# johannesulf/TabCorr

Hardware: AMD Instinct MI355X
Metric: predict_calls_per_sec (higher is better)
Workload: dtype f64; 1 GPU; BASELINE configs[1]: Zheng07 predict(), synthetic auto table 50 mass bins x {cen,sat} (G=100, P=5050), 19 rp bins, n_gauss_prim=10, batch of 10000 draws per GPU per step, draws and results resident in HBM; n_tables=1, gather=none, gather_payload=ngal + xi (160 B per draw), gather_every_steps=32, lanes=4, rccl_ranks=0

## Files before the change

tabcorr_amd/csrc/internal.h:

```cpp
#pragma once

#include <hip/hip_runtime.h>
#include <hip/hip_ext.h>

#include <algorithm>
#include <chrono>
#include <cmath>
#include <cstdarg>
#include <cstdio>
#include <cstdlib>
#include <cstring>
#include <map>
#include <memory>
#include <string>
#include <utility>
#include <vector>

#include "../../include/tabcorr_amd.h"
#include "../../include/tabcorr_amd_testing.h"
#include "fastmath.h"
#include "hostmath.h"
#include "kernel_args.h"

namespace tc {
// ... 188 lines not shown
    tried = false;
  }
};

inline int env_int(const char* name, int fallback) {
#ifdef TC_DEVELOPER_KNOBS
  const char* value = getenv(name);
  if (value == nullptr || *value == 0) return fallback;
  return atoi(value);
#else
  (void)name;
  return fallback;
#endif
}

struct Tuning {
  int lanes = 4;
  int pipeline = 1;
  int single_draw = 1;
  int many_blocks = 256;
  int single_round = 1;
  int poll_done = 1;
  int quad_waves = 0;
  int quad_waves_f32 = 3;
  int quad_merge = 1;
  int quad_order = -1;
  int prio_occ = 2, prio_contract = 1, prio_finalize = 3;
  int finalize_threads = 0;
  int finalize_row_blocks = 0;
  int occ_splits = 0;
  int occ_per_cu = 4;
  int n_groups = 0, n_waves = 0, lds_min = 0, min_chunk_entries = 32;
  int k_splits = 0;
  int trace = 0;
  int autotune_after = 0;
  int sync_chunks = 0;
  int sync_form = 32;
  int sync_stagger = 10;
  int sync_direct_out = 2;
  int async_direct_in = 1;
  int async_direct_out = 2;
  int series = -1;
  int cross_defer = 1;
  int fused_defer = 2;
  int fused_sat_cap = 6;
  int cross_wide_min_draws = 4096;
  int cross_target = 160;
  int resident_aperture = 1;
  int cross_min_draws = 192;
  int fused = 1;
  int fused_min_draws = 0;
  int fused_max_draws = 30720;
  int fused_waves = 0;
  int fused_draws = 0;
  int fused_spread = 1, fused_spread_min = 8192, fused_spread_rounds = 1;
  int prio_fused = 1, prio_fused_occ = 2, prio_fused_out = 3;
  int deterministic = 0;
  int skip_occ = 0, skip_finalize = 0;
  void load() {
    fused = env_int("TC_FUSED", fused);
    fused_min_draws = env_int("TC_FUSED_MIN_DRAWS", fused_min_draws);
    fused_max_draws = env_int("TC_FUSED_MAX_DRAWS", fused_max_draws);
    prio_fused = env_int("TC_PRIO_FUSED", prio_fused);
    prio_fused_occ = env_int("TC_PRIO_FUSED_OCC", prio_fused_occ);
    prio_fused_out = env_int("TC_PRIO_FUSED_OUT", prio_fused_out);
    lanes = env_int("TC_LANES", lanes);
    pipeline = env_int("TC_PIPELINE", pipeline);
    single_draw = env_int("TC_SINGLE_DRAW", single_draw);
    quad_waves = env_int("TC_QUAD_WAVES", quad_waves);
    quad_waves_f32 = env_int("TC_QUAD_WAVES_F32", quad_waves_f32);
    quad_merge = env_int("TC_QUAD_MERGE", quad_merge);
    prio_occ = env_int("TC_PRIO_O", prio_occ);
    prio_contract = env_int("TC_PRIO_C", prio_contract);
    prio_finalize = env_int("TC_PRIO_F", prio_finalize);
    finalize_threads = env_int("TC_FINALIZE_THREADS", finalize_threads);
    finalize_row_blocks = env_int("TC_FINALIZE_ROW_BLOCKS", finalize_row_blocks);
    occ_splits = env_int("TC_OCC_SPLITS", occ_splits);
    occ_per_cu = env_int("TC_OCC_PER_CU", occ_per_cu);
    n_groups = env_int("TC_NGROUPS", n_groups);
    n_waves = env_int("TC_NWAVES", n_waves);
    lds_min = env_int("TC_LDS_MIN", lds_min);
    min_chunk_entries = env_int("TC_MIN_CHUNK_ENTRIES", min_chunk_entries);
    k_splits = env_int("TC_KSPLITS", k_splits);
    trace = env_int("TC_TRACE", trace);
    skip_occ = env_int("TC_SKIP_OCC", skip_occ);
    skip_finalize = env_int("TC_SKIP_FINALIZE", skip_finalize);
  }
};

}
}

struct AutoChoice {
  static constexpr int kSizes = 9;
  static constexpr int64_t size(int i) { return (int64_t)256 << i; }
  int form[kSizes] = {};
  float us[kSizes][3] = {};
  int form_for(int64_t n_draws) const {
    if (n_draws <= size(0)) return form[0];
    if (n_draws >= size(kSizes - 1)) return form[kSizes - 1];
    int i = 0;
    while (size(i + 1) < n_draws) ++i;
    const double w = (double)(n_draws - size(i)) / (double)(size(i + 1) - size(i));
    static const int shape[3] = {0, 64, 32};
    int best = 0;
    double best_us = (1.0 - w) * us[i][0] + w * us[i + 1][0];
// ... 271 lines not shown
```

tabcorr_amd/csrc/kernels.hip.h:

```cpp
#pragma once

#include <hip/hip_runtime.h>

#include <cstdint>
#include <utility>

#include "fastmath.h"
#include "hostmath.h"
#include "kernel_args.h"
#include "series.h"

#ifdef TC_DEVELOPER_KNOBS
#define TC_TRACE(pointer) ((pointer) != nullptr)
#else
#define TC_TRACE(pointer) false
#endif

namespace tc {

static_assert(sizeof(QuadRun) == 32 && sizeof(QuadCompArgs) == 32, "read as 8 x int32");

typedef const __attribute__((address_space(4))) double* sc_f64;
typedef const __attribute__((address_space(4))) float* sc_f32;
typedef const __attribute__((address_space(4))) int32_t* sc_i32;
// ... 1857 lines not shown
    } else {
#pragma unroll
      for (int u = 0; u < UU; ++u) {
        const double av = u ? t.y : t.x;
        D[u][0] = __builtin_amdgcn_mfma_f64_16x16x4f64(av, b.x, D[u][0], 0, 0, 0);
        D[u][1] = __builtin_amdgcn_mfma_f64_16x16x4f64(av, b.y, D[u][1], 0, 0, 0);
      }
    }
  };
  fetch(t0, b0, cb);
  while (left > 0) {
    const int row_length = triangular ? rb + 1 : n_cb;
    const int n = row_length - cb < left ? row_length - cb : left;
    left -= n;
    f64x2 e[4];
#pragma unroll
    for (int v = 0; v < 4; ++v) e[v] = *(const f64x2*)(dens_e + (4 * rb + v) * DL);
    fetch(t1, b1, n > 1 ? cb + 1 : 0);
    __builtin_amdgcn_sched_barrier(0);
    mma(t0, b0, true);
    __builtin_amdgcn_sched_barrier(0);
    int t = 1;
    for (; t + 1 < n; t += 2) {
      fetch(t0, b0, cb + t + 1);
      __builtin_amdgcn_sched_barrier(0);
      mma(t1, b1, false);
      __builtin_amdgcn_sched_barrier(0);
      fetch(t1, b1, t + 2 < n ? cb + t + 2 : 0);
      __builtin_amdgcn_sched_barrier(0);
      mma(t0, b0, false);
      __builtin_amdgcn_sched_barrier(0);
    }
    if (t < n) {
      fetch(t0, b0, 0);
      __builtin_amdgcn_sched_barrier(0);
      mma(t1, b1, false);
      __builtin_amdgcn_sched_barrier(0);
    } else {
      t0 = t1;
      b0 = b1;
    }
#pragma unroll
    for (int u = 0; u < UU; ++u)
#pragma unroll
      for (int v = 0; v < 4; ++v) {
        F[u][0] = fma(D[u][0][v], e[v].x, F[u][0]);
        F[u][1] = fma(D[u][1][v], e[v].y, F[u][1]);
      }
    ++rb;
    cb = 0;
  }
}

__device__ __forceinline__ int wave_prefix_sum(int value) {
  auto shifted = [](int x, auto control, auto rows) {
    return __builtin_amdgcn_update_dpp(0, x, decltype(control)::value, decltype(rows)::value, 0xf,
                                       false);
  };
  typedef std::integral_constant<int, 0xf> all_rows;
  value += shifted(value, std::integral_constant<int, 0x111>(), all_rows());
  value += shifted(value, std::integral_constant<int, 0x112>(), all_rows());
  value += shifted(value, std::integral_constant<int, 0x114>(), all_rows());
  value += shifted(value, std::integral_constant<int, 0x118>(), all_rows());
  value += shifted(value, std::integral_constant<int, 0x142>(), std::integral_constant<int, 0xa>());
  value += shifted(value, std::integral_constant<int, 0x143>(), std::integral_constant<int, 0xc>());
  return value;
}

__device__ __forceinline__ double fused_quad_rows40(double select, double value, double sums) {
  return __builtin_amdgcn_mfma_f64_4x4x4f64(select, value, sums, 0, 0, 0);
}

template <int S0, int NS>
__device__ __forceinline__ void fused_quad_pass40(__amdgpu_buffer_rsrc_t rs_t, unsigned off_a,
                                                  unsigned unit_bytes, const double* dens_b,
                                                  const double* dens_e, int rb, int cb, int left,
                                                  bool triangular, int n_cb, unsigned unit_base,
                                                  double (&F)[NS][10]) {
  unsigned ua = (unit_base + (unsigned)(triangular ? rb * (rb + 1) / 2 + cb : rb * n_cb + cb)) *
                unit_bytes;
  double ta[2][NS];
  f64x2 tb[2][5];
  double D[NS][10];
  auto fetch = [&](int set, int column) {
#pragma unroll
    for (int s = 0; s < NS; ++s) {
      constexpr int kPairBytes = 1024;
      const int sub = S0 + s;
      const bool first_of_pair = (sub & 1) == 0 && s + 1 < NS;
      const bool second_of_pair = (sub & 1) == 1 && s >= 1;
      if (first_of_pair) {
        const f64x2 word = __builtin_bit_cast(
            f64x2, __builtin_amdgcn_raw_buffer_load_b128(rs_t, off_a + (sub / 2) * kPairBytes, ua,
                                                         0));
        ta[set][s] = word.x;
        ta[set][s + 1 < NS ? s + 1 : s] = word.y;
      } else if (!second_of_pair) {
        ta[set][s] = __builtin_bit_cast(
            double, __builtin_amdgcn_raw_buffer_load_b64(
                        rs_t, off_a + (sub / 2) * kPairBytes + (sub & 1) * 8, ua, 0));
      }
    }
#pragma unroll
    for (int q = 0; q < 5; ++q) tb[set][q] = *(const f64x2*)(dens_b + 4 * column * 40 + 2 * q);
    ua += unit_bytes;
  };
// ... 25 lines not shown
    const int n = row_length - cb < left ? row_length - cb : left;
    left -= n;
    f64x2 e[5];
#pragma unroll
    for (int q = 0; q < 5; ++q) e[q] = *(const f64x2*)(dens_e + 4 * rb * 40 + 2 * q);
    int t = 0;
    if (n > 1) {
      fetch(1, cb + 1);
      mma(0, true);
      fetch(0, 2 < n ? cb + 2 : 0);
      mma(1, false);
      t = 2;
    }
    for (; t + 1 < n; t += 2) {
      fetch(1, cb + t + 1);
      mma(0, false);
      fetch(0, t + 2 < n ? cb + t + 2 : 0);
      mma(1, false);
    }
    if (t < n) {
      fetch(1, 0);
      if (t == 0) mma(0, true); else mma(0, false);
#pragma unroll
      for (int s = 0; s < NS; ++s) ta[0][s] = ta[1][s];
#pragma unroll
      for (int q = 0; q < 5; ++q) tb[0][q] = tb[1][q];
    }
#pragma unroll
    for (int q = 0; q < 5; ++q)
#pragma unroll
      for (int s = 0; s < NS; ++s) {
        F[s][2 * q] = fma(D[s][2 * q], e[q].x, F[s][2 * q]);
        F[s][2 * q + 1] = fma(D[s][2 * q + 1], e[q].y, F[s][2 * q + 1]);
      }
    ++rb;
    cb = 0;
  }
}

template <int NGAUSS, int U, bool ASSEMBIAS, bool MODULATE, bool LEAUTHAUD = false,
          int W = kFusedWaves, int DL = 64, bool GROUPED = false, int SATDEFER = 0>
__global__ __launch_bounds__(64 * W, DL == 40 ? 2 : W == 8 ? (SATDEFER == 2 ? 4 : 2) : 1) void predict_fused_kernel(
    FusedArgs a) {
  static_assert(!SATDEFER || (NGAUSS == 10 && !ASSEMBIAS && !MODULATE && !LEAUTHAUD && DL != 32 &&
                              !GROUPED), "deferred pairs");
  static_assert(!GROUPED || (NGAUSS == 10 && !LEAUTHAUD), "groups of bins: Zheng07, ten nodes");
  static_assert((DL == 64 && (W == 8 || W == 16)) || ((DL == 32 || DL == 40) && W == 8),
                "workgroup shape");
  static_assert(DL == 64 || NGAUSS == 10 || LEAUTHAUD, "32 / 40 draws: ten nodes per bin");
  static_assert(DL != 40 || (!ASSEMBIAS && !MODULATE && !LEAUTHAUD && !GROUPED), "latency form");
  constexpr int PARTS = DL == 40 ? W : W * 32 / DL;
  static_assert(!LEAUTHAUD || (NGAUSS == 0 && !ASSEMBIAS), "Leauthaud11: any n_gauss, undecorated");
  constexpr int UP = (U + 1) / 2;
  extern __shared__ __attribute__((aligned(16))) double fused_lds[];
  constexpr int kSlotDoubles = fused_slot_doubles(W, DL);
  const int region_b = a.dens_rows * DL > kSlotDoubles ? a.dens_rows * DL : kSlotDoubles;
  double* dens = fused_lds;
  double* table = fused_lds + region_b;
  double(*red)[W][kLanes] = (double(*)[W][kLanes])(table + fm::kTableDoubles);
  const fm::Consts kc = fm::make_consts();
#ifdef TC_DEVELOPER_KNOBS
  const int skip = (a.priority >> 8) & 3;
  const int n_bins_occ = (skip & 1) ? 0 : a.n_bins;
  unsigned long long* const stamps =
      ((a.priority >> 10) & 1) && a.chi2 == nullptr ? (unsigned long long*)a.chi2_data : nullptr;
  auto wave_stamp = [&](int which) {
    if (stamps != nullptr && (threadIdx.x & 63) == 0 && W == 8 && ((threadIdx.x >> 6) & 3) == 0)
      stamps[blockIdx.x * 32 + 16 + 8 * (threadIdx.x >> 8) + which] =
          __builtin_amdgcn_s_memrealtime();
  };
  auto stamp = [&](int which) {
    if (stamps != nullptr && threadIdx.x == 0)
      stamps[blockIdx.x * 32 + which] = __builtin_amdgcn_s_memrealtime();
  };
  if (skip & 1)
    for (int idx = threadIdx.x; idx < a.n_bins * DL; idx += blockDim.x) fused_lds[idx] = 1e-3;
#else
  constexpr int skip = 0;
  const int n_bins_occ = a.n_bins;
  auto stamp = [](int) {};
  auto wave_stamp = [](int) {};
#endif
  stamp(0);
  set_priority((a.priority >> 2) & 3);
  const int lane = threadIdx.x & 63;
  const int wave = __builtin_amdgcn_readfirstlane(threadIdx.x >> 6);
  const int n_gauss = NGAUSS > 0 ? NGAUSS : a.n_gauss;
  {
    typedef double __attribute__((ext_vector_type(2))) double2v;
    const int hi = fm::kTableDoubles / 2;
    const double2v* src = (const double2v*)a.math_table;
    double2v* dst = (double2v*)table;
    for (int i = threadIdx.x; i < hi; i += blockDim.x) dst[i] = src[i];
  }
  for (int idx = a.n_bins * DL + threadIdx.x; idx < a.dens_rows * DL; idx += blockDim.x)
    dens[idx] = 0.0;
  __syncthreads();
  stamp(1);

  const int draw = DL != 32 ? lane : (lane & 31);
  const int half = DL != 32 ? 0 : (lane >> 5);
  const bool live = DL != 40 || lane < 40;
  auto dens_at = [&](int row, int d) -> double& {
    return dens[DL == 40 ? dens40(row, d) : row * DL + d];
  };
  const int64_t col = (int64_t)blockIdx.x * DL;
  const int64_t b0 = col + draw;
  const int64_t b = b0 < a.n_draws ? b0 : a.n_draws - 1;
  double norm;
  {
    const double* th = a.theta + b * a.n_theta;
    LeauthaudDraw ld;
    if (LEAUTHAUD) ld = prepare_leauthaud(table, kc, th);
    DrawParams dp = LEAUTHAUD ? prepare_draw(table, kc, 12.0, 1.0, 12.0, 13.0, 1.0, 0.0, 0.0)
                              : draw_params<ASSEMBIAS>(table, kc, th);
    series_setup<MODULATE>(dp, (GROUPED ? a.group.series : a.series) != nullptr && DL != 32,
                           (GROUPED ? a.group.sat_series : a.sat_series) != nullptr && DL != 32);
    sc_f64 log_m = (sc_f64)a.log_m;
    sc_f64 mass = (sc_f64)a.m;
    sc_f64 weight = (sc_f64)a.weight;
    sc_f64 weight_sum = weight + a.n_bins * n_gauss;
    sc_f64 n_h = (sc_f64)a.n_h;
    sc_f64 percentile = (sc_f64)a.percentile;
    const double f1 = (1.0 - a.split) / a.split, f2 = a.split / (1.0 - a.split);
    double sum_cen = 0.0, sum_sat = 0.0;
    stamp(2);
    if (GROUPED) {
      sc_i32 group_begin = (sc_i32)a.group.begin;
      sc_f64 n_h_m = (sc_f64)a.group.n_h;
      const GroupConsts gq{(sc_f64)a.group.log_m, (sc_f64)a.group.m, (sc_f64)a.group.weight,
                           (sc_f64)a.group.weight + a.n_bins * 10, (sc_f64)a.group.percentile,
                           (sc_i32)a.group.member,
                           SeriesConsts{(sc_f64)a.group.series, (sc_i32)a.group.series_thr,
                                        (sc_f64)a.group.sat_series,
                                        (sc_i32)a.group.sat_series_thr}};
      for (int gr = wave; gr < a.n_groups; gr += W) {
        const bool central = gr < a.n_central_groups;
        auto emit = [&](int mi, int g, double acc) {
          const double value = acc * n_h_m[mi];
          if (half == 0) dens[g * DL + draw] = value;
          if (central) sum_cen += value; else sum_sat += value;
        };
        if (DL == 32)
          occ_group_zheng07_halves<ASSEMBIAS, MODULATE>(
              table, kc, gr, group_begin[gr], group_begin[gr + 1], central, half, a.group.log_m,
              a.group.m, a.group.weight, gq, a.split, dp, emit);
        else
          occ_group_zheng07<ASSEMBIAS, MODULATE>(table, kc, gr, group_begin[gr],
                                                 group_begin[gr + 1], central, gq, a.split, dp,
                                                 emit);
      }
    }
    unsigned mine = 0;
    for (int g = wave; g < (GROUPED ? 0 : n_bins_occ); g += W) {
      const bool central = g < a.n_central;
      const bool above = ASSEMBIAS ? percentile[g] > a.split : false;
      bool deferred = false;
      const double acc =
          SATDEFER == 2 && central
              ? occ_cen_record(table, kc,
                               (sc_f64)a.cen_records + g * series::cen_record::kStride, dp,
                               &deferred) :
          SATDEFER && !central && (SATDEFER == 2 || a.sat_cap == series::sat::kShortest)
              ? occ_sat_record(table, kc,
                               (sc_f64)a.sat_records + g * series::sat_record::kStride, dp,
                               &deferred) :
          DL == 32 && LEAUTHAUD
              ? occ_bin_leauthaud11_halves<MODULATE>(table, kc, g, central, half, a.log_m, a.m,
                                                     a.weight, ld)
          : DL == 32  ? occ_bin_zheng07_halves<ASSEMBIAS, MODULATE>(table, kc, g, central, above,
                                                                    half, a.log_m, a.m, a.weight,
                                                                    log_m, weight_sum, dp)
          : LEAUTHAUD ? occ_bin_leauthaud11<MODULATE>(table, kc, g, n_gauss, central, log_m, mass,
                                                      weight, ld)
                      : occ_bin_zheng07<NGAUSS, ASSEMBIAS, MODULATE>(
                            table, kc, g, n_gauss, central, above, log_m, mass, weight,
                            weight_sum, dp, f1, f2,
                            SeriesConsts{(sc_f64)a.series, (sc_i32)a.series_thr, (sc_f64)a.sat_series,
                              (sc_i32)a.sat_series_thr,
                              SATDEFER ? a.sat_cap : series::sat::kSteps - 1},
                            SATDEFER ? &deferred : nullptr);
      if (SATDEFER && deferred && live) mine |= 1u << ((g - wave) / W);
      const double value = acc * n_h[g];
      if (half == 0 && live) dens_at(g, draw) = value;
      if (central) sum_cen += value; else sum_sat += value;
    }
    wave_stamp(0);
    if (SATDEFER) {
      unsigned* list = (unsigned*)&red[1][wave][0];
      const int count = __builtin_popcount(mine);
      const int inclusive = wave_prefix_sum(count);
      const int total = __builtin_amdgcn_readlane(inclusive, 63);
      wave_stamp(2);
      for (int base = 0; base < total; base += 64) {
        {
          unsigned left = mine;
          int position = inclusive - count - base;
          while (__builtin_amdgcn_ballot_w64(left != 0) != 0) {
            if (left != 0) {
              const int j = __builtin_ctz(left);
              left &= left - 1;
              if (position >= 0 && position < 64) list[position] = ((unsigned)j << 6) | (unsigned)lane;
              ++position;
            }
          }
        }
        wave_stamp(3);
        const int n = total - base < 64 ? total - base : 64;
        const bool active = lane < n;
        const unsigned entry = list[active ? lane : 0];
        const int g = wave + W * (int)(entry >> 6), from = (int)(entry & 63);
        const double m0 = __shfl(dp.m0, from, 64);
        const double log2_m1 = __shfl(dp.log2_m1, from, 64);
        const double sat_scale = __shfl(dp.sat_scale, from, 64);
        const double alpha = __shfl(dp.alpha, from, 64);
        const int bad = __shfl(dp.bad, from, 64);
        double acc = 0.0;
        const bool cen_pair = SATDEFER == 2 && g < a.n_central;
        if (SATDEFER == 2 && __builtin_amdgcn_ballot_w64(active && cen_pair) != 0) {
          const double log_m_min = __shfl(dp.log_m_min, from, 64);
          const double inv_sigma = __shfl(dp.inv_sigma, from, 64);
          double sum = 0.0;
          bool tie = false;
#pragma unroll 1
          for (int k0 = 0; k0 < 10; k0 += 5) {
            double node[5], w[5];
#pragma unroll
            for (int k = 0; k < 5; ++k) {
              node[k] = a.log_m[g * 10 + k0 + k];
              w[k] = a.weight[g * 10 + k0 + k];
            }
#pragma unroll
            for (int k = 0; k < 5; ++k) {
              sum = fma(w[k], fm::erf_fast(table, kc, (node[k] - log_m_min) * inv_sigma), sum);
              tie = tie || node[k] == log_m_min;
            }
          }
          sum = fma(0.5, sum, 0.5 * a.weight[a.n_bins * 10 + g]);
          if ((bad & kBadCen) || ((bad & kTieCen) && tie)) sum = __builtin_nan("");
          if (cen_pair) acc = sum;
        }
        if (SATDEFER != 2 || __builtin_amdgcn_ballot_w64(active && !cen_pair) != 0) {
        double sat = 0.0;
#pragma unroll 1
        for (int k0 = 0; k0 < 10; k0 += 5) {
          double node[5], w[5];
#pragma unroll
          for (int k = 0; k < 5; ++k) {
            node[k] = a.m[g * 10 + k0 + k];
            w[k] = a.weight[g * 10 + k0 + k];
          }
#pragma unroll
          for (int k = 0; k < 5; ++k) {
            const double x = node[k] - m0;
            sat = fma(w[k],
                      fm::exp2_fast(table, kc,
                                    alpha * fm::log2_fast_offset(
                                                table, kc, x > 1e-300 ? x : 1e-300, log2_m1),
                                    x > 0.0),
                      sat);
          }
        }
        sat *= sat_scale;
        if (bad != 0) {
          if ((bad & kInfSat) && sat != 0.0) sat = __builtin_huge_val();
          if ((bad & kBadSat) && sat != 0.0) sat = __builtin_nan("");
        }
        if (!cen_pair) acc = sat;
        }
        if (active) dens_at(g, from) = acc * a.n_h[g];
        wave_stamp(4);
      }
      for (unsigned left = mine; __builtin_amdgcn_ballot_w64(left != 0) != 0;) {
        if (left != 0) {
          const int j = __builtin_ctz(left);
          left &= left - 1;
          const double value = dens_at(wave + W * j, draw);
          if (SATDEFER == 2 && wave + W * j < a.n_central) sum_cen += value;
          else sum_sat += value;
        }
      }
    }
    wave_stamp(1);
    stamp(3);
    red[0][wave][lane] = sum_cen;
    red[1][wave][lane] = sum_sat;
    __syncthreads();
    stamp(4);
    double n_cen = 0.0, n_sat = 0.0;
#pragma unroll
    for (int w = 0; w < W; ++w) {
      n_cen += red[0][w][lane];
      n_sat += red[1][w][lane];
    }
    const double total = (skip & 1) ? 1.0 : n_cen + n_sat;
    norm = total * total;
    if (wave == 0 && half == 0 && live && b0 < a.n_draws) {
      if (a.separate) {
        a.ngal[2 * b0] = n_cen;
        a.ngal[2 * b0 + 1] = n_sat;
      } else {
        a.ngal[b0] = total;
      }
    }
  }

  set_priority(a.priority & 3);
  const int c = lane & 15, kq = lane >> 4;
  double F[UP][2][2];
  constexpr int UA = DL == 40 ? (U > 3 ? 3 : U) : 1, UB = DL == 40 && U > 3 ? U - 3 : 1;
  double F40a[UA][10], F40b[UB][10];
  if (DL == 40) {
    const int part = wave;
    const unsigned off_a = ((lane & 0x30) | ((lane & 3) << 2) | ((lane >> 2) & 3)) * 16;
    const double* dens_b = dens + (a.part_j_row0[part] + (lane >> 4)) * 40 + (lane & 3) * 10;
    const double* dens_e = dens + (a.part_i_row0[part] + (lane >> 4)) * 40 + (lane & 3) * 10;
    const __amdgpu_buffer_rsrc_t rs_t =
        __builtin_amdgcn_make_buffer_rsrc((void*)a.table, 0, a.table_bytes, kBufferFlags);
    const int rb = a.part_rb0[part], cb = a.part_cb0[part], count = a.part_count[part];
    const bool triangular = a.part_triangular[part] != 0;
    const int n_cb = a.part_n_cb[part];
    const unsigned unit_base = (unsigned)a.part_unit_base[part];
#pragma unroll
    for (int s = 0; s < UA; ++s)
#pragma unroll
      for (int g = 0; g < 10; ++g) F40a[s][g] = 0.0;
#pragma unroll
    for (int s = 0; s < UB; ++s)
#pragma unroll
      for (int g = 0; g < 10; ++g) F40b[s][g] = 0.0;
#ifdef TC_DEVELOPER_KNOBS
    const unsigned unit_bytes = ((a.priority >> 12) & 1) ? 0u : UP * 1024u;
    const unsigned first_unit = ((a.priority >> 12) & 1) ? 0u : unit_base;
#else
    constexpr unsigned unit_bytes = UP * 1024u;
    const unsigned first_unit = unit_base;
#endif
    if (!(skip & 2))
    fused_quad_pass40<0, UA>(rs_t, off_a, unit_bytes, dens_b, dens_e, rb, cb, count, triangular,
                             n_cb, first_unit, F40a);
    if (U > 3 && !(skip & 2))
      fused_quad_pass40<(U > 3 ? 3 : 0), UB>(rs_t, off_a, unit_bytes, dens_b, dens_e, rb, cb,
                                             count, triangular, n_cb, first_unit, F40b);
  } else {
    const int sub = wave / PARTS, part = wave % PARTS;
    const unsigned off_a = lane * 16;
    const double* dens_b =
        dens + (a.part_j_row0[part] + kq) * DL + sub * kQuadTile + 2 * c;
    const double* dens_e = dens + a.part_i_row0[part] * DL + sub * kQuadTile + 2 * c;
    const __amdgpu_buffer_rsrc_t rs_t =
        __builtin_amdgcn_make_buffer_rsrc((void*)a.table, 0, a.table_bytes, kBufferFlags);
    const int rb = a.part_rb0[part], cb = a.part_cb0[part], count = a.part_count[part];
    const bool triangular = a.part_triangular[part] != 0;
    const int n_cb = a.part_n_cb[part];
    const unsigned unit_base = (unsigned)a.part_unit_base[part];
#pragma unroll
    for (int p = 0; p < UP; ++p) {
      F[p][0][0] = F[p][0][1] = F[p][1][0] = F[p][1][1] = 0.0;
      if (skip & 2) continue;
      if (2 * p + 1 < U)
        fused_quad_pass<2, DL>(rs_t, off_a + p * 1024, UP * 1024, dens_b, dens_e, rb, cb, count,
                               triangular, n_cb, unit_base, F[p]);
      else
        fused_quad_pass<1, DL>(rs_t, off_a + p * 1024, UP * 1024, dens_b, dens_e, rb, cb, count,
                               triangular, n_cb, unit_base, F[p]);
    }
  }
  stamp(5);
  __syncthreads();
  stamp(8);
  if (DL == 40) {
    const int q = lane >> 4;
    auto share = [&](int sub, int g) {
      return sub < UA ? F40a[sub < UA ? sub : 0][g] : F40b[sub >= UA ? sub - UA : 0][g];
    };
    double* out = dens + (wave * (4 * U) + ((lane >> 2) & 3)) * 40 + (lane & 3);
    if (((a.priority >> 11) & 1) && __builtin_amdgcn_ballot_w64(!(norm < 1e280)) == 0) {
      double select[4];
#pragma unroll
      for (int m = 0; m < 4; ++m) select[m] = (lane & 3) == m ? 1.0 : 0.0;
#pragma unroll
      for (int sub = 0; sub < U; ++sub)
#pragma unroll
        for (int t = 0; t < 3; ++t) {
          double sums = 0.0;
#pragma unroll
          for (int m = 0; m < (t < 2 ? 4 : 2); ++m)
            sums = fused_quad_rows40(select[m], share(sub, 4 * t + m), sums);
          if (t < 2 || q < 2) out[(4 * sub) * 40 + 16 * t + 4 * q] = sums;
        }
    } else {
#pragma unroll
      for (int sub = 0; sub < U; ++sub)
#pragma unroll
        for (int g = 0; g < 10; ++g) {
          const double sum = fused_quad_rows40(1.0, share(sub, g), 0.0);
          if (q == 0) out[(4 * sub) * 40 + 4 * g] = sum;
        }
    }
  } else {
    double* out = dens + (wave * (4 * U) + kq) * kQuadTile + 2 * c;
#pragma unroll
    for (int u = 0; u < U; ++u) {
      const f64x2 value = {F[u >> 1][u & 1][0], F[u >> 1][u & 1][1]};
      *(f64x2*)(out + (4 * u) * kQuadTile) = value;
    }
  }
  stamp(9);
  set_priority((a.priority >> 4) & 3);
  double(*tile)[kLanes + 1] = (double(*)[kLanes + 1])table;
  if (a.separate) {
    const bool poisoned = !(fabs(norm) <= 1.79769313486231570815e308);
    const int64_t n_valid = a.n_draws - col < DL ? a.n_draws - col : DL;
    const int sub = lane >> 5, d = lane & 31;
    for (int comp = 0; comp < 3; ++comp) {
      __syncthreads();
      constexpr int Q = PARTS / 4;
      const int p_begin = comp == 0 ? 0 : comp == 1 ? Q : 3 * Q;
      const int p_count = comp == 1 ? 2 * Q : Q;
      for (int rr = wave; rr < a.n_r && lane < DL; rr += W) {
        const double* first = dens + ((PARTS * sub + p_begin) * (4 * U) + rr) * kQuadTile + d;
        double sum = first[0];
        for (int p = 1; p < p_count; ++p) sum += first[p * (4 * U) * kQuadTile];
        tile[rr][lane] = poisoned ? __builtin_nan("") : sum / norm;
      }
      __syncthreads();
      for (int idx = threadIdx.x; idx < a.n_r * DL; idx += blockDim.x) {
        const int dd = idx / a.n_r, rr = idx % a.n_r;
        if (dd < n_valid) a.xi[((col + dd) * 3 + comp) * (int64_t)a.n_r + rr] = tile[rr][dd];
      }
    }
    return;
  }
  double* chi2_lds = table + 20 * (kLanes + 1);
  if (a.chi2 != nullptr) {
    const int count = a.n_r * (a.n_r + 1);
    for (int idx = threadIdx.x; idx < count; idx += blockDim.x) chi2_lds[idx] = a.chi2_data[idx];
  }
  __syncthreads();
  stamp(10);
  if (DL == 40) {
    for (int rr = wave; rr < a.n_r && lane < DL; rr += W) {
      const double* first = dens + rr * 40 + lane;
      double sum = first[0];
#pragma unroll
      for (int part = 1; part < W; ++part) sum += first[part * (4 * U) * 40];
      tile[rr][lane] = sum / norm;
    }
  } else {
    const int sub = lane >> 5, d = lane & 31;
    for (int rr = wave; rr < a.n_r && lane < DL; rr += W) {
      const double* first = dens + ((PARTS * sub) * (4 * U) + rr) * kQuadTile + d;
      double sum = first[0];
#pragma unroll
      for (int part = 1; part < PARTS; ++part) sum += first[part * (4 * U) * kQuadTile];
      tile[rr][lane] = sum / norm;
    }
  }
  __syncthreads();
  stamp(6);
  const int64_t n_valid = a.n_draws - col < DL ? a.n_draws - col : DL;
  if (a.chi2 != nullptr) {
    const int rows = a.n_r;
    const double* data = chi2_lds;
    const double* matrix = chi2_lds + rows;
    double part = 0.0;
    for (int i = wave; i < rows; i += W) {
      double inner = 0.0;
      for (int j = 0; j < rows; ++j)
        inner = fma(matrix[i * rows + j], tile[j][lane] - data[j], inner);
      part = fma(tile[i][lane] - data[i], inner, part);
    }
    red[0][wave][lane] = part;
    __syncthreads();
    if (wave == 0 && lane < n_valid) {
      double total = 0.0;
      for (int w = 0; w < W; ++w) total += red[0][w][lane];
      a.chi2[col + lane] = total;
    }
    return;
  }
  for (int idx = threadIdx.x; idx < a.n_r * DL; idx += blockDim.x) {
    const int d = idx / a.n_r, rr = idx % a.n_r;
    if (d < n_valid) a.xi[(col + d) * (int64_t)a.n_r + rr] = tile[rr][d];
  }
  stamp(7);
}

template <int ROW_LANES, typename Coefficient>
__device__ __forceinline__ void cross_deferred_pairs(
    const CrossFusedArgs& a, const double* table, const fm::Consts& kc, const DrawParams& dp,
    const unsigned long long* bitmap, unsigned* list, int wave, int lane, int g_first, int g_last,
    int type, Coefficient&& coefficient, double* res) {
  constexpr int SHARES = 64 / ROW_LANES;
  constexpr int SLOTS = 8 / SHARES;
  const int row = lane % ROW_LANES, share = lane / ROW_LANES;
  const unsigned long long owner = 0x0101010101010101ull << wave;
  double extra[SLOTS];
#pragma unroll
  for (int slot = 0; slot < SLOTS; ++slot) extra[slot] = 0.0;
  auto evaluate = [&](int total) {
#ifdef TC_DEVELOPER_KNOBS
    if (((a.priority >> 10) & 1) && a.chi2 == nullptr && lane == 0) {
// ... 1783 lines not shown
```

tabcorr_amd/csrc/launch.hip:

```cpp
#include <immintrin.h>

#include <atomic>
#include <mutex>

#include "internal.h"
#include "kernels.hip.h"
#include "series.h"

namespace tc {
namespace host {

int get_quadrature(tc_table* t, int n_gauss, Quadrature** out) {
  auto it = t->quadrature.find(n_gauss);
  if (it != t->quadrature.end()) {
    *out = &it->second;
    return TC_OK;
  }
  std::vector<double> x, w;
  tc::gauss_legendre(n_gauss, x, w);
  const int g = t->n_bins;
  std::vector<double> log_m((size_t)g * n_gauss), m((size_t)g * n_gauss),
      weight((size_t)g * n_gauss + g);
  for (int i = 0; i < g; ++i) {
    const double d_log = t->log_max[i] - t->log_min[i];
// ... 916 lines not shown
  fa.n_theta = n_theta;
  fa.n_bins = t->n_bins;
  fa.n_central = t->plan.n_central;
  fa.n_gauss = n_gauss;
  fa.dens_rows = fused_dens_rows(t, separate);
  fa.separate = separate ? 1 : 0;
  const bool spread = fused_spread_eligible(t, n_draws, n_gauss, flags);
  const bool wide = !spread && fused_wide_tables(t, separate, n_gauss, flags);
  const bool half_tiles = !spread && !wide && fused_half_tiles(t, separate, n_draws, n_gauss, flags);
  const int waves = spread || wide || half_tiles ? 8 : fused_waves(t, separate, flags);
  const int draws = spread ? 40 : wide || half_tiles ? 32 : 64;
  const int n_parts = spread ? 8 : waves * 32 / draws;
  if (!separate) {
    const tc::QuadComp& comp = q_table.layout.comps[0];
    tc::triangle_parts(comp.n_rb, n_parts, fa.part_rb0, fa.part_cb0, fa.part_count);
    for (int part = 0; part < n_parts; ++part) {
      fa.part_triangular[part] = 1;
      fa.part_n_cb[part] = comp.n_cb;
      fa.part_i_row0[part] = comp.i_bin0;
      fa.part_j_row0[part] = comp.j_bin0;
      fa.part_unit_base[part] = (int)comp.unit_base;
    }
  } else {
    const int quarter = n_parts / 4;
    for (int part = 0; part < n_parts; ++part) {
      const int c = part < quarter ? 0 : part < 3 * quarter ? 1 : 2;
      const int first = c == 0 ? 0 : c == 1 ? quarter : 3 * quarter;
      const int pieces = c == 1 ? 2 * quarter : quarter, piece = part - first;
      const tc::QuadComp& comp = q_table.layout.comps[c];
      fa.part_triangular[part] = comp.triangular;
      fa.part_n_cb[part] = comp.n_cb;
      fa.part_i_row0[part] = comp.i_bin0;
      fa.part_j_row0[part] = comp.j_bin0;
      fa.part_unit_base[part] = (int)comp.unit_base;
      if (comp.triangular) {
        int32_t rb0[tc::kFusedMaxParts], cb0[tc::kFusedMaxParts], count[tc::kFusedMaxParts];
        tc::triangle_parts(comp.n_rb, pieces, rb0, cb0, count);
        fa.part_rb0[part] = rb0[piece];
        fa.part_cb0[part] = cb0[piece];
        fa.part_count[part] = count[piece];
      } else {
        const int64_t begin = comp.n_units * piece / pieces;
        const int64_t end = comp.n_units * (piece + 1) / pieces;
        fa.part_rb0[part] = (int)(begin / comp.n_cb);
        fa.part_cb0[part] = (int)(begin % comp.n_cb);
        fa.part_count[part] = (int)(end - begin);
      }
    }
  }
  fa.n_r = t->n_r;
  fa.priority = (t->tuning.prio_fused & 3) | ((t->tuning.prio_fused_occ & 3) << 2) |
                ((t->tuning.prio_fused_out & 3) << 4) |
                ((env_int_early("TC_FUSED_SKIP", 0) & 3) << 8) |
                (q_table.finite ? 1 << 11 : 0);
  fa.n_draws = n_draws;
  fa.n_groups = t->node_groups.n_groups;
  fa.n_central_groups = t->node_groups.n_central_groups;
  fa.group = group_args(t, *q);
  fa.series = (series_mask(t) & 1) ? (const double*)q->series : nullptr;
  fa.series_thr = (const int32_t*)q->series_thr;
  fa.sat_series = (series_mask(t) & 2) ? (const double*)q->sat_series : nullptr;
  fa.sat_series_thr = (const int32_t*)q->sat_series_thr;
  fa.log_m = (const double*)q->log_m;
  fa.m = (const double*)q->m;
  fa.weight = (const double*)q->weight;
  fa.n_h = (const double*)t->d_n_h;
  fa.percentile = (const double*)t->d_percentile;
  fa.split = 0.5;
  fa.math_table = (const double*)t->d_math_table;
  fa.table = q_table.d_table;
  fa.table_bytes =
      (uint32_t)((size_t)q_table.layout.n_units * (size_t)((t->quad_tiling.n_u + 1) / 2) * 1024);
  fa.ngal = ngal_device;
  fa.xi = xi_device;
  t->chi2_fused = false;
  if (t->fuse_chi2_out != nullptr) {
    fa.chi2_data = t->fuse_chi2_data;
    fa.chi2 = t->fuse_chi2_out;
    fa.xi = nullptr;
    t->chi2_fused = true;
  }
  const int lds = fused_lds_bytes(t, separate, waves, draws);
  const dim3 grid((unsigned)((n_draws + draws - 1) / draws)), block(64 * waves);
#ifdef TC_DEVELOPER_KNOBS
  if (fa.chi2 == nullptr && env_int_early("TC_FUSED_STAMPS", 0) != 0) {
    t->trace_blocks = ((size_t)grid.x * 32 + 5) / 6;
    status = t->trace.reserve(t->trace_blocks * 6 * sizeof(unsigned long long), stream);
    if (status != TC_OK) return status;
    fa.chi2_data = (const double*)t->trace.ptr;
    fa.priority |= 1 << 10;
  }
  if (env_int_early("TC_FUSED_SAME_UNIT", 0) != 0) fa.priority |= 1 << 12;
#endif
  hipEvent_t k0 = nullptr, k1 = nullptr;
  status = next_kernel_events(t, &k0, &k1);
  if (status != TC_OK) return status;
  const bool assembias = (flags & TC_FLAG_ASSEMBIAS) != 0;
  const bool modulate = (flags & TC_FLAG_MODULATE_WITH_CENOCC) != 0;
  const bool sat_defer = t->tuning.fused_defer != 0 && !assembias && !modulate &&
                         !(flags & TC_FLAG_LEAUTHAUD11) && n_gauss == 10 && !wide &&
                         !half_tiles && waves == 8 && t->n_bins <= 256 &&
                         !(t->grouped && n_gauss == 10) && t->tuning.series != 0 &&
                         q->sat_series != nullptr && q->sat_records != nullptr;
  if (sat_defer) fa.sat_series = (const double*)q->sat_series;
  fa.sat_records = (const double*)q->sat_records;
  fa.cen_records = (const double*)q->cen_records;
  const bool cen_defer = sat_defer && t->tuning.fused_defer >= 2 && (series_mask(t) & 1) != 0 &&
// ... 956 lines not shown
```

tabcorr_amd/csrc/table.cpp:

```cpp
#include <cmath>

#include "internal.h"

using namespace tc::host;

extern "C" {

int tc_table_create(int mode, int n_bins, int n_r, int64_t n_pairs,
                    const void* tpcf_matrix, int matrix_dtype, const double* n_h,
                    const double* log_min, const double* log_max,
                    const double* percentile, const double* dist_index,
                    const uint8_t* is_central, int compute_dtype, tc_table** out) {
  TC_CHECK(out != nullptr, "table output pointer is NULL");
  *out = nullptr;
  TC_CHECK(mode == TC_MODE_AUTO || mode == TC_MODE_CROSS, "invalid mode %d", mode);
  TC_CHECK(n_bins >= 1 && n_bins < (1 << 20), "invalid number of bins %d", n_bins);
  TC_CHECK(n_r >= 1, "invalid number of correlation function bins %d", n_r);
  const int64_t expect =
      mode == TC_MODE_AUTO ? (int64_t)n_bins * (n_bins + 1) / 2 : n_bins;
  TC_CHECK(n_pairs == expect,
           "tpcf_matrix has %lld columns but %d bins in mode '%s' need %lld",
           (long long)n_pairs, n_bins, mode == TC_MODE_AUTO ? "auto" : "cross",
           (long long)expect);
  TC_CHECK(n_pairs < (1LL << 31), "too many pair columns");
// ... 1319 lines not shown
  } else if (key == "sync_chunks") {
    TC_CHECK(value >= -1 && value <= 64, "sync_chunks must be in [-1, 64]");
    t->tuning.sync_chunks = value;
  } else if (key == "sync_stagger") {
    TC_CHECK(value >= 0 && value <= 100, "sync_stagger must be in [0, 100]");
    t->tuning.sync_stagger = value;
  } else if (key == "sync_form") {
    TC_CHECK(value == 0 || value == 32 || value == 64, "sync_form must be 0, 32 or 64");
    t->tuning.sync_form = value;
  } else if (key == "sync_direct_out") {
    TC_CHECK(value >= 0 && value <= 2, "sync_direct_out must be 0, 1 or 2");
    t->tuning.sync_direct_out = value;
  } else if (key == "async_direct_in" || key == "async_direct_out") {
    (key == "async_direct_in" ? t->tuning.async_direct_in : t->tuning.async_direct_out) =
        value;
  } else if (key == "fused") {
    TC_CHECK(value >= 0 && value <= 2, "fused must be 0, 1 or 2");
    t->tuning.fused = value;
  } else if (key == "fused_min_draws" || key == "fused_max_draws") {
    TC_CHECK(value >= (key == "fused_min_draws" ? 0 : 1), "%s must be positive", name);
    (key == "fused_min_draws" ? t->tuning.fused_min_draws : t->tuning.fused_max_draws) = value;
  } else if (key == "resident") {
    TC_CHECK(value >= 0 && value <= 2, "resident must be 0, 1 or 2");
    t->resident.enabled = value == 1;
    t->resident.auto_mode = value == 2;
    t->resident.auto_streak = t->resident.auto_backoff = 0;
    t->resident.auto_window = t->resident.auto_relaunches = 0;
    t->resident.auto_failures = 0;
    t->resident.ens_disabled = false;
    t->resident.ens_failures = 0;
    if (value != 1) return resident_stop(t);
  } else if (key == "resident_inject_failures") {
    TC_CHECK(value >= 0, "resident_inject_failures must not be negative");
    t->resident.inject_failures = value;
  } else if (key == "resident_auto_idle_us") {
    TC_CHECK(value >= 10 && value <= 100000, "resident_auto_idle_us must be in [10, 100000]");
    const int status = resident_stop(t);
    if (status != TC_OK) return status;
    t->resident.auto_idle_us = value;
  } else if (key == "resident_poll_waves") {
    TC_CHECK(value >= 1 && value <= 4, "resident_poll_waves must be in [1, 4]");
    const int status = resident_stop(t);
    if (status != TC_OK) return status;
    t->resident.poll_waves = value;
  } else if (key == "resident_idle_us") {
    TC_CHECK(value >= 10 && value <= 1000000, "resident_idle_us must be in [10, 1000000]");
    const int status = resident_stop(t);
    if (status != TC_OK) return status;
    t->resident.idle_us = value;
  } else if (key == "fused_draws") {
    TC_CHECK(value == 0 || value == 32 || value == 40 || value == 64,
             "fused_draws must be 0, 32, 40 or 64");
    t->tuning.fused_draws = value;
  } else if (key == "fused_spread") {
    t->tuning.fused_spread = value != 0;
  } else if (key == "fused_spread_min") {
    TC_CHECK(value >= 1, "fused_spread_min must be positive");
    t->tuning.fused_spread_min = value;
  } else if (key == "fused_spread_rounds") {
    TC_CHECK(value >= 1 && value <= 64, "fused_spread_rounds must be in [1, 64]");
    t->tuning.fused_spread_rounds = value;
  } else if (key == "fused_waves") {
    TC_CHECK(value == 0 || value == 8 || value == 16, "fused_waves must be 0, 8 or 16");
    t->tuning.fused_waves = value;
  } else if (key == "prio_fused") {
    t->tuning.prio_fused = value & 3;
  } else if (key == "prio_fused_occ") {
    t->tuning.prio_fused_occ = value & 3;
  } else if (key == "prio_fused_out") {
    t->tuning.prio_fused_out = value & 3;
  } else if (key == "single_draw") {
    t->tuning.single_draw = value != 0;
  } else if (key == "many_blocks") {
    TC_CHECK(value >= 2 && value <= 4096, "many_blocks must be in [2, 4096]");
    t->tuning.many_blocks = value;
  } else if (key == "single_round") {
    t->tuning.single_round = value != 0;
  } else if (key == "poll_done") {
    t->tuning.poll_done = value != 0;
  } else if (key == "trace") {
    t->tuning.trace = value;
  } else if (key == "occ_splits" || key == "occ_per_cu" || key == "finalize_threads" ||
             key == "finalize_row_blocks") {
    TC_CHECK(value >= 0 && value <= 4096, "invalid value");
    (key == "occ_splits" ? t->tuning.occ_splits
     : key == "occ_per_cu" ? t->tuning.occ_per_cu
     : key == "finalize_threads" ? t->tuning.finalize_threads
                                 : t->tuning.finalize_row_blocks) = value;
  } else if (key == "prio_occ" || key == "prio_contract" || key == "prio_finalize") {
    TC_CHECK(value >= 0 && value <= 3, "priorities are 0..3");
    (key == "prio_occ" ? t->tuning.prio_occ
                       : key == "prio_contract" ? t->tuning.prio_contract
                                                : t->tuning.prio_finalize) = value;
  } else if (key == "quad_merge" || key == "quad_waves" || key == "quad_order") {
    for (tc_table::Lane& lane : t->lanes)
      if (lane.stream) TC_HIP(hipStreamSynchronize(lane.stream));
    if (key == "quad_merge") t->tuning.quad_merge = value != 0;
    else if (key == "quad_order") t->tuning.quad_order = value;
    else t->tuning.quad_waves = t->tuning.quad_waves_f32 = value;
    for (tc::host::QuadTable* q : {&t->quad_by_type, &t->quad_total}) q->drop_schedules();
  } else {
    return fail(TC_ERR_INVALID, "unknown option '%s'", name);
  }
  return TC_OK;
}

// ... 93 lines not shown
```

Baseline: 271.9 million calls/s.

## Skip all-zero density blocks in fused quadratic pass by sorting draws by cutoff

Reorders draws within each 64-draw workgroup by how many satellite mass bins fall below their mass cutoff, so draws with similar zero patterns share a 32-draw half. Per-wave ballots then mark 4-row density blocks that are zero for every draw, and a new quad pass iterates only over non-zero tile units via bitmasks, skipping their MFMAs and table loads. The pass is rotated across waves by block index to spread load. Adds ballot and mask bookkeeping overhead, disables skipping when totals are non-finite, and only applies to the 8-wave, 64-draw, non-separate configuration.

```diff
diff --git a/tabcorr_amd/csrc/internal.h b/tabcorr_amd/csrc/internal.h
--- a/tabcorr_amd/csrc/internal.h
+++ b/tabcorr_amd/csrc/internal.h
@@ -264,6 +264,7 @@
   int fused_min_draws = 0;
   int fused_max_draws = 30720;
   int fused_waves = 0;
+  int fused_skip = 1;
   int fused_draws = 0;
   int fused_spread = 1, fused_spread_min = 8192, fused_spread_rounds = 1;
   int prio_fused = 1, prio_fused_occ = 2, prio_fused_out = 3;
diff --git a/tabcorr_amd/csrc/kernels.hip.h b/tabcorr_amd/csrc/kernels.hip.h
--- a/tabcorr_amd/csrc/kernels.hip.h
+++ b/tabcorr_amd/csrc/kernels.hip.h
@@ -1933,6 +1933,120 @@
   }
 }
 
+struct FusedZeroBlocks {
+  unsigned long long set0, set1;
+};
+
+template <int UU>
+__device__ __forceinline__ void fused_quad_pass_skip(__amdgpu_buffer_rsrc_t rs_t, unsigned off_a,
+                                                     unsigned unit_bytes, const double* dens_b,
+                                                     const double* dens_e, int rb, int cb, int left,
+                                                     bool triangular, int n_cb, unsigned unit_base,
+                                                     const FusedZeroBlocks zero, double (&F)[2][2]) {
+  constexpr int DL = 64;
+  typedef unsigned long long mask_t;
+  struct Unit {
+    int row;
+    bool on0, on1, first0, first1, last;
+  };
+  mask_t todo0 = 0, todo1 = 0;
+  bool fresh0 = true, fresh1 = true;
+  int row = rb - 1, cb_lo = cb;
+  f64x4 D[UU][2];
+  auto next_row = [&]() {
+    while (left > 0) {
+      ++row;
+      const int row_length = triangular ? row + 1 : n_cb;
+      const int n = row_length - cb_lo < left ? row_length - cb_lo : left;
+      left -= n;
+      const mask_t range = (n >= 64 ? ~0ull : (1ull << n) - 1ull) << cb_lo;
+      cb_lo = 0;
+      todo0 = ((zero.set0 >> row) & 1ull) ? 0ull : range & ~zero.set0;
+      todo1 = ((zero.set1 >> row) & 1ull) ? 0ull : range & ~zero.set1;
+      fresh0 = fresh1 = true;
+      if ((todo0 | todo1) != 0ull) return true;
+    }
+    return false;
+  };
+  auto pop = [&](Unit& u, f64x2& t, f64x2& b) {
+    if ((todo0 | todo1) == 0ull && !next_row()) return false;
+    const int column = __builtin_ctzll(todo0 | todo1);
+    const mask_t bit = 1ull << column;
+    u.row = row;
+    u.on0 = (todo0 & bit) != 0ull;
+    u.on1 = (todo1 & bit) != 0ull;
+    u.first0 = fresh0;
+    u.first1 = fresh1;
+    fresh0 = fresh0 && !u.on0;
+    fresh1 = fresh1 && !u.on1;
+    todo0 &= ~bit;
+    todo1 &= ~bit;
+    u.last = (todo0 | todo1) == 0ull;
+    const unsigned ua =
+        (unit_base + (unsigned)(triangular ? row * (row + 1) / 2 + column : row * n_cb + column)) *
+        unit_bytes;
+    t = buffer_load16<0>(rs_t, off_a, ua);
+    b = *(const f64x2*)(dens_b + 4 * column * DL);
+    return true;
+  };
+  auto run = [&](const Unit& u, const f64x2& t, const f64x2& b) {
+    f64x2 e[4];
+    if (u.last) {
+#pragma unroll
+      for (int v = 0; v < 4; ++v) e[v] = *(const f64x2*)(dens_e + (4 * u.row + v) * DL);
+    }
+    __builtin_amdgcn_sched_barrier(0);
+    const f64x4 none = {0.0, 0.0, 0.0, 0.0};
+    if (u.on0) {
+      if (u.first0) {
+#pragma unroll
+        for (int k = 0; k < UU; ++k)
+          D[k][0] = __builtin_amdgcn_mfma_f64_16x16x4f64(k ? t.y : t.x, b.x, none, 0, 0, 0);
+      } else {
+#pragma unroll
+        for (int k = 0; k < UU; ++k)
+          D[k][0] = __builtin_amdgcn_mfma_f64_16x16x4f64(k ? t.y : t.x, b.x, D[k][0], 0, 0, 0);
+      }
+    }
+    if (u.on1) {
+      if (u.first1) {
+#pragma unroll
+        for (int k = 0; k < UU; ++k)
+          D[k][1] = __builtin_amdgcn_mfma_f64_16x16x4f64(k ? t.y : t.x, b.y, none, 0, 0, 0);
+      } else {
+#pragma unroll
+        for (int k = 0; k < UU; ++k)
+          D[k][1] = __builtin_amdgcn_mfma_f64_16x16x4f64(k ? t.y : t.x, b.y, D[k][1], 0, 0, 0);
+      }
+    }
+    __builtin_amdgcn_sched_barrier(0);
+    if (u.last) {
+      if (u.on0 || !u.first0) {
+#pragma unroll
+        for (int k = 0; k < UU; ++k)
+#pragma unroll
+          for (int v = 0; v < 4; ++v) F[k][0] = fma(D[k][0][v], e[v].x, F[k][0]);
+      }
+      if (u.on1 || !u.first1) {
+#pragma unroll
+        for (int k = 0; k < UU; ++k)
+#pragma unroll
+          for (int v = 0; v < 4; ++v) F[k][1] = fma(D[k][1][v], e[v].y, F[k][1]);
+      }
+    }
+  };
+  Unit u0, u1;
+  f64x2 t0, t1, b0, b1;
+  bool more = pop(u0, t0, b0);
+  while (more) {
+    more = pop(u1, t1, b1);
+    run(u0, t0, b0);
+    if (!more) break;
+    more = pop(u0, t0, b0);
+    run(u1, t1, b1);
+  }
+}
+
 __device__ __forceinline__ int wave_prefix_sum(int value) {
   auto shifted = [](int x, auto control, auto rows) {
     return __builtin_amdgcn_update_dpp(0, x, decltype(control)::value, decltype(rows)::value, 0xf,
@@ -2064,6 +2178,7 @@
   constexpr int PARTS = DL == 40 ? W : W * 32 / DL;
   static_assert(!LEAUTHAUD || (NGAUSS == 0 && !ASSEMBIAS), "Leauthaud11: any n_gauss, undecorated");
   constexpr int UP = (U + 1) / 2;
+  constexpr bool SKIPPABLE = W == 8 && DL == 64 && !LEAUTHAUD;
   extern __shared__ __attribute__((aligned(16))) double fused_lds[];
   constexpr int kSlotDoubles = fused_slot_doubles(W, DL);
   const int region_b = a.dens_rows * DL > kSlotDoubles ? a.dens_rows * DL : kSlotDoubles;
@@ -2120,6 +2235,10 @@
   const int64_t b0 = col + draw;
   const int64_t b = b0 < a.n_draws ? b0 : a.n_draws - 1;
   double norm;
+  int column = draw;
+  bool skipping = false, unsafe = false;
+  if constexpr (SKIPPABLE)
+    skipping = ((a.priority >> 13) & 1) && !a.separate && a.dens_rows <= 256;
   {
     const double* th = a.theta + b * a.n_theta;
     LeauthaudDraw ld;
@@ -2136,6 +2255,30 @@
     sc_f64 percentile = (sc_f64)a.percentile;
     const double f1 = (1.0 - a.split) / a.split, f2 = a.split / (1.0 - a.split);
     double sum_cen = 0.0, sum_sat = 0.0;
+    if constexpr (SKIPPABLE) {
+      if (skipping) {
+        typedef unsigned long long mask_t;
+        const mask_t regular = __builtin_amdgcn_ballot_w64(dp.bad == 0);
+        mask_t alive = ~0ull;
+        int rank = 0, base = 0;
+        for (int g = a.n_central; g <= a.n_bins && alive != 0ull; ++g) {
+          mask_t below = 0ull;
+          if (g < a.n_bins) {
+            const double m_a = mass[g * n_gauss], m_b = mass[g * n_gauss + n_gauss - 1];
+            below = __builtin_amdgcn_ballot_w64(!((m_a > m_b ? m_a : m_b) > dp.m0)) & regular;
+          }
+          const mask_t leaving = alive & ~below;
+          alive &= below;
+          if (leaving != 0ull) {
+            const int before = __builtin_amdgcn_mbcnt_hi(
+                (unsigned)(leaving >> 32), __builtin_amdgcn_mbcnt_lo((unsigned)leaving, 0));
+            if ((leaving >> lane) & 1ull) rank = base + before;
+            base += __builtin_popcountll(leaving);
+          }
+        }
+        column = ((rank >> 5) << 5) | ((rank & 15) << 1) | ((rank >> 4) & 1);
+      }
+    }
     stamp(2);
     if (GROUPED) {
       sc_i32 group_begin = (sc_i32)a.group.begin;
@@ -2150,7 +2293,7 @@
         const bool central = gr < a.n_central_groups;
         auto emit = [&](int mi, int g, double acc) {
           const double value = acc * n_h_m[mi];
-          if (half == 0) dens[g * DL + draw] = value;
+          if (half == 0) dens[g * DL + (SKIPPABLE ? column : draw)] = value;
           if (central) sum_cen += value; else sum_sat += value;
         };
         if (DL == 32)
@@ -2194,7 +2337,7 @@
                             SATDEFER ? &deferred : nullptr);
       if (SATDEFER && deferred && live) mine |= 1u << ((g - wave) / W);
       const double value = acc * n_h[g];
-      if (half == 0 && live) dens_at(g, draw) = value;
+      if (half == 0 && live) dens_at(g, SKIPPABLE ? column : draw) = value;
       if (central) sum_cen += value; else sum_sat += value;
     }
     wave_stamp(0);
@@ -2280,14 +2423,14 @@
         }
         if (!cen_pair) acc = sat;
         }
-        if (active) dens_at(g, from) = acc * a.n_h[g];
+        if (active) dens_at(g, SKIPPABLE ? __shfl(column, from, 64) : from) = acc * a.n_h[g];
         wave_stamp(4);
       }
       for (unsigned left = mine; __builtin_amdgcn_ballot_w64(left != 0) != 0;) {
         if (left != 0) {
           const int j = __builtin_ctz(left);
           left &= left - 1;
-          const double value = dens_at(wave + W * j, draw);
+          const double value = dens_at(wave + W * j, SKIPPABLE ? column : draw);
           if (SATDEFER == 2 && wave + W * j < a.n_central) sum_cen += value;
           else sum_sat += value;
         }
@@ -2307,6 +2450,7 @@
     }
     const double total = (skip & 1) ? 1.0 : n_cen + n_sat;
     norm = total * total;
+    if constexpr (SKIPPABLE) unsafe = dp.bad != 0 || !(fabs(total) < 1e140);
     if (wave == 0 && half == 0 && live && b0 < a.n_draws) {
       if (a.separate) {
         a.ngal[2 * b0] = n_cen;
@@ -2320,6 +2464,7 @@
   set_priority(a.priority & 3);
   const int c = lane & 15, kq = lane >> 4;
   double F[UP][2][2];
+  int slot = wave;
   constexpr int UA = DL == 40 ? (U > 3 ? 3 : U) : 1, UB = DL == 40 && U > 3 ? U - 3 : 1;
   double F40a[UA][10], F40b[UB][10];
   if (DL == 40) {
@@ -2355,7 +2500,10 @@
       fused_quad_pass40<(U > 3 ? 3 : 0), UB>(rs_t, off_a, unit_bytes, dens_b, dens_e, rb, cb,
                                              count, triangular, n_cb, first_unit, F40b);
   } else {
-    const int sub = wave / PARTS, part = wave % PARTS;
+    const int sub = wave / PARTS;
+    const int part = SKIPPABLE && skipping ? (wave + 3 * sub + (int)blockIdx.x) % PARTS
+                                           : wave % PARTS;
+    if constexpr (SKIPPABLE) slot = sub * PARTS + part;
     const unsigned off_a = lane * 16;
     const double* dens_b =
         dens + (a.part_j_row0[part] + kq) * DL + sub * kQuadTile + 2 * c;
@@ -2366,10 +2514,38 @@
     const bool triangular = a.part_triangular[part] != 0;
     const int n_cb = a.part_n_cb[part];
     const unsigned unit_base = (unsigned)a.part_unit_base[part];
+    FusedZeroBlocks zero{0ull, 0ull};
+    if constexpr (SKIPPABLE) {
+      if (skipping && ((a.priority >> 11) & 1)) {
+        const int n_blocks = a.dens_rows / 4;
+        const double* block = dens + kq * DL + sub * kQuadTile + 2 * c;
+        for (int k = 0; k < n_blocks; ++k) {
+          const f64x2 value = *(const f64x2*)(block + 4 * k * DL);
+          if (__builtin_amdgcn_ballot_w64(value.x != 0.0) == 0ull) zero.set0 |= 1ull << k;
+          if (__builtin_amdgcn_ballot_w64(value.y != 0.0) == 0ull) zero.set1 |= 1ull << k;
+        }
+        const bool mine = (column >> 5) == sub;
+        if (__builtin_amdgcn_ballot_w64(unsafe && mine && (column & 1) == 0) != 0ull)
+          zero.set0 = 0ull;
+        if (__builtin_amdgcn_ballot_w64(unsafe && mine && (column & 1) == 1) != 0ull)
+          zero.set1 = 0ull;
+      }
+    }
 #pragma unroll
     for (int p = 0; p < UP; ++p) {
       F[p][0][0] = F[p][0][1] = F[p][1][0] = F[p][1][1] = 0.0;
       if (skip & 2) continue;
+      if constexpr (SKIPPABLE) {
+        if (skipping) {
+          if (2 * p + 1 < U)
+            fused_quad_pass_skip<2>(rs_t, off_a + p * 1024, UP * 1024, dens_b, dens_e, rb, cb,
+                                    count, triangular, n_cb, unit_base, zero, F[p]);
+          else
+            fused_quad_pass_skip<1>(rs_t, off_a + p * 1024, UP * 1024, dens_b, dens_e, rb, cb,
+                                    count, triangular, n_cb, unit_base, zero, F[p]);
+          continue;
+        }
+      }
       if (2 * p + 1 < U)
         fused_quad_pass<2, DL>(rs_t, off_a + p * 1024, UP * 1024, dens_b, dens_e, rb, cb, count,
                                triangular, n_cb, unit_base, F[p]);
@@ -2411,7 +2587,7 @@
         }
     }
   } else {
-    double* out = dens + (wave * (4 * U) + kq) * kQuadTile + 2 * c;
+    double* out = dens + (slot * (4 * U) + kq) * kQuadTile + 2 * c;
 #pragma unroll
     for (int u = 0; u < U; ++u) {
       const f64x2 value = {F[u >> 1][u & 1][0], F[u >> 1][u & 1][1]};
@@ -2460,7 +2636,8 @@
       tile[rr][lane] = sum / norm;
     }
   } else {
-    const int sub = lane >> 5, d = lane & 31;
+    const int at = SKIPPABLE ? column : lane;
+    const int sub = at >> 5, d = at & 31;
     for (int rr = wave; rr < a.n_r && lane < DL; rr += W) {
       const double* first = dens + ((PARTS * sub) * (4 * U) + rr) * kQuadTile + d;
       double sum = first[0];
diff --git a/tabcorr_amd/csrc/launch.hip b/tabcorr_amd/csrc/launch.hip
--- a/tabcorr_amd/csrc/launch.hip
+++ b/tabcorr_amd/csrc/launch.hip
@@ -992,7 +992,8 @@
   fa.priority = (t->tuning.prio_fused & 3) | ((t->tuning.prio_fused_occ & 3) << 2) |
                 ((t->tuning.prio_fused_out & 3) << 4) |
                 ((env_int_early("TC_FUSED_SKIP", 0) & 3) << 8) |
-                (q_table.finite ? 1 << 11 : 0);
+                (q_table.finite ? 1 << 11 : 0) |
+                (t->tuning.fused_skip && !separate && waves == 8 && draws == 64 ? 1 << 13 : 0);
   fa.n_draws = n_draws;
   fa.n_groups = t->node_groups.n_groups;
   fa.n_central_groups = t->node_groups.n_central_groups;
diff --git a/tabcorr_amd/csrc/table.cpp b/tabcorr_amd/csrc/table.cpp
--- a/tabcorr_amd/csrc/table.cpp
+++ b/tabcorr_amd/csrc/table.cpp
@@ -1395,6 +1395,8 @@
     TC_CHECK(value == 0 || value == 32 || value == 40 || value == 64,
              "fused_draws must be 0, 32, 40 or 64");
     t->tuning.fused_draws = value;
+  } else if (key == "fused_skip") {
+    t->tuning.fused_skip = value != 0;
   } else if (key == "fused_spread") {
     t->tuning.fused_spread = value != 0;
   } else if (key == "fused_spread_min") {
```

After: 205.9 million calls/s. 0.757x the previous value.
